# ahcorde/visualSLAM_Android

Measured on AMD Instinct MI355X. Metric: frames/sec (TrackFrame+local BA) on 640×480 synthetic, 1/2/4/8 GPU, higher is better.
Workload: dtype f64

## Files before the change

### include/vslam_c.h

```cpp
#ifndef VSLAM_C_H
#define VSLAM_C_H

#include <stddef.h>
#include <stdint.h>

#ifdef __cplusplus
extern "C" {
#endif

#define VSLAM_LEVELS 4

#define VSLAM_OK 0
#define VSLAM_E_INVALID (-1)
#define VSLAM_E_HIP (-2)
#define VSLAM_E_CAPACITY (-3)
#define VSLAM_E_STATE (-4)

#define VSLAM_Q_CAM_INT_RADIUS 1
#define VSLAM_Q_POSE_INT_RESIDUAL 2
#define VSLAM_Q_NONMAX_RIGHT_NEIGHBOUR 4

typedef struct vslam_system vslam_system;

typedef struct vslam_params {
// ... 32 lines not shown
  int bootstrap;
  int ba_sum_order;
  int relocalise;
  double reloc_blur;
  unsigned pvs_shuffle_seed;
  int overlay;
  int keyframe_retire;
} vslam_params;

const char* vslam_last_error(void);
int vslam_default_params(vslam_params* p, int width, int height, int n_streams);

int vslam_create(const vslam_params* p, vslam_system** out);
int vslam_destroy(vslam_system* sys);
int vslam_synchronize(vslam_system* sys);
int vslam_eval_transcendental(int fn, int n, const double* x, double* y, int on_host);
int vslam_eval_select(int form, int n, const double* v, int k, double* out);
int vslam_eval_pose_tail(const double* sums27, const double* pose12, double* update6, double* pose12_out);


int vslam_make_keyframe_lite(vslam_system* sys, const uint8_t* gray, size_t row_stride,
                             size_t stream_stride, int on_device);

int vslam_fast_nonmax(vslam_system* sys);

int vslam_read_level_image(vslam_system* sys, int stream, int level, uint8_t* dst, size_t dst_stride);
int vslam_read_corners(vslam_system* sys, int stream, int level, uint32_t* corners ,
                       int cap, int* n);
int vslam_read_row_lut(vslam_system* sys, int stream, int level, int* lut );
int vslam_read_max_corners(vslam_system* sys, int stream, int level, uint32_t* corners, int* scores,
                           int cap, int* n);

int vslam_make_keyframe_rest(vslam_system* sys, double min_shi_tomasi_score);
int vslam_thin_candidates(vslam_system* sys, int keyframe);
int vslam_read_candidates(vslam_system* sys, int stream, int level, uint32_t* pos, double* score, int cap, int* n);
int vslam_get_keyframe_corners(vslam_system* sys, int stream, int keyframe, int level, uint32_t* corners, int cap, int* n);
int vslam_read_sbi(vslam_system* sys, int stream, uint8_t* small_img, float* tmpl, double rot8[8]);
int vslam_read_keyframe_sbi(vslam_system* sys, int stream, int keyframe, float* tmpl, float* jacs);
int vslam_get_reloc_info(vslam_system* sys, int stream, int out_i[4], double out_d[24]);
int vslam_read_reloc_attempt(vslam_system* sys, int stream, float* cur_tmpl, double* zmssd, int cap);

int vslam_minipatch_sample(vslam_system* sys, int stream, int n, const int* pos_xy, uint8_t* patches , int* ok);
int vslam_minipatch_find(vslam_system* sys, int stream, int n, const uint8_t* patches, int* pos_xy, int range, int max_ssd,
                         int* found);


// ... 182 lines not shown
```

### visualslam_android_amd/capi.py

```python
import threading
import ctypes as C
import os

import numpy as np

LEVELS = 4
N_STAGES = 14
_HERE = os.path.dirname(os.path.abspath(__file__))
LIB_PATH = os.path.join(_HERE, "libvslam_hip.so")

Q_CAM_INT_RADIUS = 1
Q_POSE_INT_RESIDUAL = 2
Q_NONMAX_RIGHT_NEIGHBOUR = 4

DRAW_POINTS = 1
DRAW_TRAILS = 2
DRAW_FAST = 4
DRAW_IN_PLACE = 8
DRAW_ALPHA0 = 16


class VslamError(RuntimeError):
    pass

# ... 42 lines not shown


class PlaneProbe(C.Structure):
    _fields_ = [("have", C.c_int), ("n", C.c_int), ("best_trial", C.c_int), ("reserved", C.c_int), ("sums", C.c_double * 100),
                ("mean", C.c_double * 3), ("normal", C.c_double * 3), ("R", C.c_double * 9), ("t", C.c_double * 3)]


_lib = None

_ip = C.POINTER(C.c_int)
_sys = C.c_void_p
_vp = C.c_void_p
_i, _d, _sz = C.c_int, C.c_double, C.c_size_t
SYMBOLS = {
    "vslam_last_error": (C.c_char_p, []),
    "vslam_default_params": (_i, [C.POINTER(Params), _i, _i, _i]),
    "vslam_create": (_i, [C.POINTER(Params), C.POINTER(_sys)]),
    "vslam_destroy": (_i, [_sys]),
    "vslam_synchronize": (_i, [_sys]),
    "vslam_eval_transcendental": (_i, [_i, _i, _vp, _vp, _i]),
    "vslam_eval_select": (_i, [_i, _i, _vp, _i, _vp]),
    "vslam_eval_pose_tail": (_i, [_vp, _vp, _vp, _vp]),
    "vslam_make_keyframe_lite": (_i, [_sys, _vp, _sz, _sz, _i]),
    "vslam_fast_nonmax": (_i, [_sys]),
    "vslam_read_level_image": (_i, [_sys, _i, _i, _vp, _sz]),
    "vslam_read_corners": (_i, [_sys, _i, _i, _vp, _i, _ip]),
    "vslam_read_row_lut": (_i, [_sys, _i, _i, _vp]),
    "vslam_read_max_corners": (_i, [_sys, _i, _i, _vp, _vp, _i, _ip]),
    "vslam_get_keyframe_corners": (_i, [_sys, _i, _i, _i, _vp, _i, _ip]),
    "vslam_read_sbi": (_i, [_sys, _i, _vp, _vp, _vp]),
    "vslam_read_keyframe_sbi": (_i, [_sys, _i, _i, _vp, _vp]),
    "vslam_get_reloc_info": (_i, [_sys, _i, _vp, _vp]),
    "vslam_read_reloc_attempt": (_i, [_sys, _i, _vp, _vp, _i]),
    "vslam_attempt_recovery": (_i, [_sys]),
    "vslam_make_keyframe_rest": (_i, [_sys, C.c_double]),
    "vslam_thin_candidates": (_i, [_sys, _i]),
    "vslam_read_candidates": (_i, [_sys, _i, _i, _vp, _vp, _i, _ip]),
    "vslam_minipatch_sample": (_i, [_sys, _i, _i, _vp, _vp, _vp]),
    "vslam_minipatch_find": (_i, [_sys, _i, _i, _vp, _vp, _i, _i, _vp]),
    "vslam_add_keyframe": (_i, [_sys, _i]),
    "vslam_map_add_keyframe": (_i, [_sys, _i, _vp, _i, _vp, _sz, _d, _d]),
    "vslam_map_add_keyframes": (_i, [_sys, _i, _i, _vp, _vp, _vp, _sz, _sz, _vp]),
    "vslam_map_add_point": (_i, [_sys, _i, _vp, _i, _i, _i, _i, _vp, _vp]),
    "vslam_map_add_points": (_i, [_sys, _i, _i, _vp, _vp, _vp, _vp, _vp, _vp]),
    "vslam_map_add_measurement": (_i, [_sys, _i, _i, _i, _i, _vp, _i, _i]),
    "vslam_map_add_measurements": (_i, [_sys, _i, _i, _vp, _vp, _vp, _vp, _vp, _vp]),
# ... 156 lines not shown


def eval_transcendental(name, x, on_host=False):
    x = _f64(x).reshape(-1)
    y = np.zeros_like(x)
    _check(load_library().vslam_eval_transcendental(TRANSCENDENTALS.index(name), len(x), x.ctypes.data, y.ctypes.data, int(on_host)))
    return y


def eval_select(v, k, form=0):
    v = _f64(v).reshape(-1)
    out = np.zeros(1)
    _check(load_library().vslam_eval_select(int(form), len(v), v.ctypes.data, int(k), out.ctypes.data))
    return out[0]


def eval_pose_tail(sums27, pose12):
    s, p = _f64(sums27).reshape(27), _f64(pose12).reshape(12)
    up, out = np.zeros(6), np.zeros(12)
    _check(load_library().vslam_eval_pose_tail(s.ctypes.data, p.ctypes.data, up.ctypes.data, out.ctypes.data))
    return up, out


def pvs_permutation(seed, frame, lst, n, keys=None, on_host=False):
    out = np.zeros(max(n, 0), np.int32)
    k = None if keys is None else np.ascontiguousarray(keys, np.uint32)
    assert k is None or len(k) == n
    _check(load_library().vslam_pvs_permutation(seed, frame, lst, n, None if k is None else k.ctypes.data, out.ctypes.data, int(on_host)))
    return out


def _prims(a, per):
    a = np.ascontiguousarray(np.zeros((0, per)) if a is None else a, np.int32).reshape(-1, per)
    return a, (a.ctypes.data if len(a) else None)


def eval_overlay(gray, marks=None, lines=None, discs=None, flags=0, rgba=None, row_stride=None):
    gray = np.ascontiguousarray(gray, np.uint8)
    h, w = gray.shape
    stride = 4 * w if row_stride is None else int(row_stride)
    nbytes = stride * (h - 1) + 4 * w
    if rgba is None:
        out = np.zeros(nbytes, np.uint8)
    else:
        out = np.ascontiguousarray(rgba, np.uint8).reshape(-1).copy()
        assert out.size >= nbytes, (out.size, nbytes)
# ... 57 lines not shown
        idx, g = self._subset(streams, gray)
        _check(self.lib.vslam_make_keyframe_lite_subset(self.h, idx.ctypes.data if len(idx) else None, len(idx),
                                                        g.ctypes.data if len(idx) else None, g.shape[2], g.shape[1] * g.shape[2], 0))
        self.synchronize()

    def make_keyframe_lite_subset_device(self, streams, dev_ptr, row_stride, stream_stride):
        idx = np.ascontiguousarray(streams, dtype=np.int32).reshape(-1)
        _check(self.lib.vslam_make_keyframe_lite_subset(self.h, idx.ctypes.data if len(idx) else None, len(idx), dev_ptr, row_stride, stream_stride, 1))

    def track_frame_subset(self, streams, gray):
        idx, g = self._subset(streams, gray)
        _check(self.lib.vslam_track_frame_subset(self.h, idx.ctypes.data if len(idx) else None, len(idx),
                                                 g.ctypes.data if len(idx) else None, g.shape[2], g.shape[1] * g.shape[2], 0))
        self.synchronize()

    def track_frame_subset_device(self, streams, dev_ptr, row_stride, stream_stride):
        idx = np.ascontiguousarray(streams, dtype=np.int32).reshape(-1)
        _check(self.lib.vslam_track_frame_subset(self.h, idx.ctypes.data if len(idx) else None, len(idx), dev_ptr, row_stride, stream_stride, 1))

    def step_streams(self):
        out = np.zeros(self.S, dtype=np.uint8)
        _check(self.lib.vslam_get_step_streams(self.h, out.ctypes.data))
        return out

    def fast_nonmax(self):
        _check(self.lib.vslam_fast_nonmax(self.h))

    def read_level_image(self, stream, level):
        h, w = self.level_shape(level)
        out = np.empty((h, w), dtype=np.uint8)
        _check(self.lib.vslam_read_level_image(self.h, stream, level, out.ctypes.data, w))
        return out

    def read_corners(self, stream, level):
        cap = self.params.max_corners[level]
        out = np.empty(cap, dtype=np.uint32)
        n = C.c_int(0)
        _check(self.lib.vslam_read_corners(self.h, stream, level, out.ctypes.data, cap, C.byref(n)))
        return out[:n.value].copy()

    def read_row_lut(self, stream, level):
        h, _ = self.level_shape(level)
        out = np.empty(h, dtype=np.int32)
        _check(self.lib.vslam_read_row_lut(self.h, stream, level, out.ctypes.data))
        return out

# ... 501 lines not shown
```

### visualslam_android_amd/csrc/frontend.hip

```cpp
#include "vslam_internal.h"
#include "fast_reject_dev.h"
#include <stdlib.h>
#include <stdio.h>

#define BAND 16
#define HALO 3
#define FE_THREADS 256

struct FeArgs {
  const uint8_t* in; size_t in_sstride; int in_pitch;
  uint8_t* lvl[NLEV]; size_t lvl_sstride[NLEV]; int lvl_pitch[NLEV];
  int w[NLEV], h[NLEV], nchunk[NLEV], thr[NLEV], cap[NLEV];
  unsigned long long* cmask[NLEV];
  int* rowcnt[NLEV];
  int* rowlut[NLEV];
  uint32_t* corners[NLEV];
  int* ncorners;
  int* overflow;
  int band_first[NLEV];
  const int* list;
};
DEVFN int fe_stream_of(const FeArgs& a, int i) { return a.list ? a.list[i] : i; }

__device__ __forceinline__ bool ring_run10(unsigned m16) {
  unsigned m = m16 | (m16 << 16);
  unsigned r2 = m & (m >> 1);
// ... 162 lines not shown
  if ((int)blockIdx.x >= a.band_first[2]) l = 2;
  if ((int)blockIdx.x >= a.band_first[3]) l = 3;
  const int b = blockIdx.x - a.band_first[l], s = fe_stream_of(a, blockIdx.y);
  const int lp = (a.w[l] + 15) & ~15;
  uint8_t* t = lds;
  unsigned long long* mask_lds = (unsigned long long*)(((uintptr_t)(t + (BAND + 2 * HALO) * lp) + 15) & ~(uintptr_t)15);
  unsigned short* cand = (unsigned short*)(mask_lds + BAND * a.nchunk[l]);
  int* ncand = (int*)(cand + FB_ROWS * lp);
  const int y0 = b * BAND;
  stage_rows(t, lp, a.lvl[l] + (size_t)s * a.lvl_sstride[l], a.lvl_pitch[l], a.w[l], a.h[l], y0 - HALO, BAND + 2 * HALO);
  __syncthreads();
  const int nrows = min(BAND, a.h[l] - y0);
  fast_band(t, lp, y0, nrows, a.w[l], a.h[l], a.thr[l], a.nchunk[l],
            a.cmask[l] + (size_t)s * a.h[l] * a.nchunk[l], a.rowcnt[l] + (size_t)s * a.h[l], mask_lds, cand, ncand);
}

#define SL_RMAX 64
#define SL_THREADS 256
#define SL_CAP 1024
#define SL_RING 8
#define SL_AHEAD (SL_RING - 7)

struct SlArgs {
  int w16[NLEV], nb[NLEV], bpw[NLEV], wg_first[NLEV + 1];
  int R[NLEV];
  int S;
};

DEVFN unsigned sl_half2(unsigned wa, unsigned wb) {
  const unsigned q0 = __builtin_amdgcn_perm(wb, wa, 0x05040100u), q1 = __builtin_amdgcn_perm(wb, wa, 0x07060302u);
  return (__builtin_amdgcn_sad_u8(q0, 0u, 2u) >> 2) | ((__builtin_amdgcn_sad_u8(q1, 0u, 2u) >> 2) << 8);
}
DEVFN unsigned sl_half4(unsigned a0, unsigned a1, unsigned b0, unsigned b1) { return sl_half2(a0, b0) | (sl_half2(a1, b1) << 16); }

struct __attribute__((packed, aligned(4))) SlRow3 { unsigned x, y, z; };
DEVFN bool sl_full_test(const uint8_t* img, int pitch, int w, int x, int y, int thr) {
  const int xb = (x - 3) & ~3, o = (x - 3) & 3;
  const int xl = min(xb, w - 12);
  const bool late = xl != xb;
  unsigned A[7], B[7], v0[7], v1[7], v2[7];
  const uint8_t* r = img + (size_t)(y - 3) * pitch + xl;
#pragma unroll
  for (int k = 0; k < 7; k++) {
    const SlRow3 v = *(const SlRow3*)r;
    v0[k] = v.x; v1[k] = v.y; v2[k] = v.z;
    r += pitch;
  }
  asm volatile("" : "+v"(v0[0]), "+v"(v0[1]), "+v"(v0[2]), "+v"(v0[3]), "+v"(v0[4]), "+v"(v0[5]), "+v"(v0[6]),
                    "+v"(v1[0]), "+v"(v1[1]), "+v"(v1[2]), "+v"(v1[3]), "+v"(v1[4]), "+v"(v1[5]), "+v"(v1[6]));
  asm volatile("" : "+v"(v2[0]), "+v"(v2[1]), "+v"(v2[2]), "+v"(v2[3]), "+v"(v2[4]), "+v"(v2[5]), "+v"(v2[6]));
#pragma unroll
  for (int k = 0; k < 7; k++) {
    const unsigned lo = late ? v1[k] : v0[k], mid = late ? v2[k] : v1[k];
    A[k] = __builtin_amdgcn_alignbyte(mid, lo, o);
    B[k] = __builtin_amdgcn_alignbyte(v2[k], mid, o);
  }
  const int c = (A[3] >> 24) & 255u, cb = c + thr, c_b = c - thr;
  unsigned mb = 0, md = 0;
#define SLPIX(k, dx, dy) { const int v = (int)(((dx) <= 0 ? (A[(dy) + 3] >> (8 * ((dx) + 3))) : (B[(dy) + 3] >> (8 * ((dx) - 1)))) & 255u); mb = __builtin_amdgcn_alignbit(mb, (unsigned)(cb - v), 31); md = __builtin_amdgcn_alignbit(md, (unsigned)(v - c_b), 31); }
  SLPIX(15, -1, 3) SLPIX(14, -2, 2) SLPIX(13, -3, 1) SLPIX(12, -3, 0) SLPIX(11, -3, -1) SLPIX(10, -2, -2)
  SLPIX(9, -1, -3) SLPIX(8, 0, -3) SLPIX(7, 1, -3) SLPIX(6, 2, -2) SLPIX(5, 3, -1) SLPIX(4, 3, 0)
  SLPIX(3, 3, 1) SLPIX(2, 2, 2) SLPIX(1, 1, 3) SLPIX(0, 0, 3)
#undef SLPIX
  return ring_run10(mb) || ring_run10(md);
}

template <bool PYR>
__global__ __launch_bounds__(SL_THREADS) __attribute__((amdgpu_waves_per_eu(4, 4))) void k_fast_slide(FeArgs a, SlArgs q) {
  extern __shared__ __align__(16) uint8_t lds[];
  int l = 0;
  if (!PYR) { l = 1; if ((int)blockIdx.x >= q.wg_first[2]) l = 2; if ((int)blockIdx.x >= q.wg_first[3]) l = 3; }
  const int wg = (int)blockIdx.x - (PYR ? 0 : q.wg_first[l]);
  const int w = a.w[l], h = a.h[l], nchunk = a.nchunk[l], thr = a.thr[l];
  const int W16 = q.w16[l], nb = q.nb[l], bpw = q.bpw[l], SL_R = q.R[l], SL_NSTEP = SL_R + 2 * HALO;
  const uint8_t* img = PYR ? a.in : a.lvl[l];
  const size_t sstride = PYR ? a.in_sstride : a.lvl_sstride[l];
  const int pitch = PYR ? a.in_pitch : a.lvl_pitch[l];
  int4* tb = (int4*)lds;
  unsigned short* lists = (unsigned short*)(tb + SL_THREADS);
  unsigned long long* mask = (unsigned long long*)(lists + (SL_THREADS / 64) * SL_CAP);
  const int tid = threadIdx.x, lane = tid & 63, wave = tid >> 6;
  unsigned short* list = lists + wave * SL_CAP;
  const int bl = tid / W16, cg = tid - bl * W16;
  const long gband = (long)wg * bpw + bl;
  const bool active = bl < bpw && gband < (long)q.S * nb;
  const int ord = active ? (int)(gband / nb) : 0, b = active ? (int)(gband - (long)ord * nb) : 0;
  const int s = active ? fe_stream_of(a, ord) : 0;
  const int yb = b * SL_R, x0 = cg * 16;
  tb[tid] = make_int4(s, yb, x0, active ? bl : -1);
  for (int i = tid; i < bpw * SL_R * nchunk; i += SL_THREADS) mask[i] = 0ull;
  __syncthreads();
  const uint8_t* base = img + (size_t)s * sstride + x0;
  unsigned xvalid = 0;
  for (int j = 0; j < 16; j++) if (x0 + j >= HALO && x0 + j < w - HALO) xvalid |= 1u << j;
  if (!active) xvalid = 0;
// ... 430 lines not shown
}

static void fill_fe_args(vslam_system* sys, FeArgs& a) {
  for (int l = 0; l < NLEV; l++) {
    a.lvl[l] = sys->d_lvl[l];
    a.lvl_sstride[l] = (size_t)sys->geom[l].pitch * sys->geom[l].h;
    a.lvl_pitch[l] = sys->geom[l].pitch;
    a.w[l] = sys->geom[l].w; a.h[l] = sys->geom[l].h; a.nchunk[l] = sys->geom[l].nchunk;
    a.thr[l] = sys->geom[l].thr; a.cap[l] = sys->geom[l].cap;
    a.cmask[l] = sys->fr.cmask[l]; a.rowcnt[l] = sys->fr.rowcnt[l]; a.rowlut[l] = sys->fr.rowlut[l];
    a.corners[l] = sys->fr.corners[l];
  }
  a.ncorners = sys->fr.ncorners;
  a.overflow = sys->fr.overflow;
  a.list = nullptr;
}

static bool fe_slide_ok(const vslam_system* sys, const FeArgs& a) {
  static const bool off = getenv("VSLAM_FE_BANDS") != nullptr;
  if (off) return false;
  for (int l = 0; l < NLEV; l++) if ((a.w[l] & 3) || a.w[l] < 16 || a.w[l] > 4096 || a.h[l] < 7) return false;
  return (((uintptr_t)a.in) & 15) == 0 && (a.in_pitch & 15) == 0 && (a.in_sstride & 15) == 0 && a.in_pitch >= ((a.w[0] + 15) & ~15);
}
static void fe_launch_slide(vslam_system* sys, FeArgs& a, hipStream_t fs, int S) {
  SlArgs q;
  q.S = S;
  int nwg[NLEV];
  size_t lds[NLEV];
  const long slots = 4L * (sys->n_cu > 0 ? sys->n_cu : 256);
  for (int l = 0; l < NLEV; l++) { q.w16[l] = (a.w[l] + 15) >> 4; q.bpw[l] = SL_THREADS / q.w16[l]; }
  auto pick = [&](int l0, int l1) {
    long best = -1; int bestR = 32;
    for (int R = 16; R <= SL_RMAX; R += 8) {
      long wgs = 0;
      bool fits = true;
      for (int l = l0; l <= l1; l++) {
        wgs += ((long)S * ((a.h[l] + R - 1) / R) + q.bpw[l] - 1) / q.bpw[l];
        if ((size_t)SL_THREADS * 16 + (size_t)(SL_THREADS / 64) * SL_CAP * 2 + (size_t)q.bpw[l] * R * a.nchunk[l] * 8 > 60000) fits = false;
      }
      if (!fits && R > 16) continue;
      const long cost = ((wgs + slots - 1) / slots) * (R + 2 * HALO);
      if (best < 0 || cost < best) { best = cost; bestR = R; }
    }
    for (int l = l0; l <= l1; l++) q.R[l] = bestR;
  };
  pick(0, 0);
  pick(1, NLEV - 1);
  for (int l = 0; l < NLEV; l++) {
    q.nb[l] = (a.h[l] + q.R[l] - 1) / q.R[l];
    nwg[l] = (int)(((long)S * q.nb[l] + q.bpw[l] - 1) / q.bpw[l]);
    lds[l] = (size_t)SL_THREADS * 16 + (size_t)(SL_THREADS / 64) * SL_CAP * 2 + (size_t)q.bpw[l] * q.R[l] * a.nchunk[l] * 8;
  }
  static const bool dbg = getenv("VSLAM_FE_DEBUG") != nullptr;
  if (dbg) fprintf(stderr, "fe slide: S %d n_cu %d R %d %d %d %d nb %d %d %d %d wgs %d %d %d %d lds %zu %zu %zu %zu\n", S, sys->n_cu, q.R[0], q.R[1], q.R[2], q.R[3],
                   q.nb[0], q.nb[1], q.nb[2], q.nb[3], nwg[0], nwg[1], nwg[2], nwg[3], lds[0], lds[1], lds[2], lds[3]);
  q.wg_first[0] = 0; q.wg_first[1] = 0;
  for (int l = 1; l < NLEV; l++) q.wg_first[l + 1] = q.wg_first[l] + nwg[l];
  size_t lds123 = lds[1]; if (lds[2] > lds123) lds123 = lds[2]; if (lds[3] > lds123) lds123 = lds[3];
  prof_mark(sys, PROF_PYR_FAST0);
  hipLaunchKernelGGL(k_fast_slide<true>, dim3(nwg[0]), dim3(SL_THREADS), lds[0], fs, a, q);
  prof_mark(sys, PROF_FAST_LVL);
  hipLaunchKernelGGL(k_fast_slide<false>, dim3(q.wg_first[NLEV]), dim3(SL_THREADS), lds123, fs, a, q);
}

#define FE_LDS_MAX (160 * 1024)
static int fe_band_lds(const void* kernel, size_t lds) {
  if (lds > FE_LDS_MAX) { vslam_set_error("front end: a band of %zu B does not fit the %d B of LDS", lds, FE_LDS_MAX); return VSLAM_E_INVALID; }
  if (lds > 48 * 1024) HIPCHK(hipFuncSetAttribute(kernel, hipFuncAttributeMaxDynamicSharedMemorySize, (int)lds));
  return VSLAM_OK;
}
static int fe_launch_bands(vslam_system* sys, FeArgs& a, hipStream_t stream, int S, bool marks) {
  const LevelGeom* g = sys->geom;
  const int lp0 = (g[0].w + 15) & ~15, lp1 = (g[1].w + 15) & ~15, lp2 = (g[2].w + 15) & ~15;
  const size_t lds0 = (size_t)(BAND + 2 * HALO) * lp0 + (BAND / 2) * lp1 + (BAND / 4) * lp2 + 16 + (size_t)BAND * g[0].nchunk * 8 + (size_t)FB_ROWS * lp0 * 2 + 16;
  const size_t lds1 = (size_t)(BAND + 2 * HALO) * lp1 + 16 + (size_t)BAND * g[1].nchunk * 8 + (size_t)FB_ROWS * lp1 * 2 + 16;
  int r = fe_band_lds((const void*)k_pyr_fast0, lds0);
  if (!r) r = fe_band_lds((const void*)k_fast_lvl, lds1);
  if (r) return r;
  if (marks) prof_mark(sys, PROF_PYR_FAST0);
  hipLaunchKernelGGL(k_pyr_fast0, dim3((g[0].h + BAND - 1) / BAND, S), dim3(FE_THREADS), lds0, stream, a, lp0, lp1, lp2);
  int nb = 0;
  a.band_first[0] = 0;
  for (int l = 1; l < NLEV; l++) { a.band_first[l] = nb; nb += (g[l].h + BAND - 1) / BAND; }
  if (marks) prof_mark(sys, PROF_FAST_LVL);
  hipLaunchKernelGGL(k_fast_lvl, dim3(nb, S), dim3(FE_THREADS), lds1, stream, a);
// ... 57 lines not shown
  } else {
    if (sys->step_subset) sys->step_in.assign((size_t)sys->S, 1);
    sys->fe_held = nullptr; sys->map.held = nullptr;
  }
  sys->step_subset = subset;
  if (on_device && !subset) {
    a.in = gray; a.in_sstride = stream_stride; a.in_pitch = (int)row_stride;
  } else {
    for (int i = 0; i < S && !on_device; i++) {
      const int s = subset ? streams[i] : i;
      HIPCHK(hipMemcpy2DAsync(sys->d_lvl[0] + (size_t)s * a.lvl_sstride[0], g[0].pitch, gray + (size_t)i * stream_stride,
                              row_stride, g[0].w, g[0].h, hipMemcpyHostToDevice, fs));
    }
    if (on_device && S > 0)
      hipLaunchKernelGGL(k_gather_level0, dim3((g[0].h + GATHER_ROWS - 1) / GATHER_ROWS, S), dim3(FE_THREADS), 0, fs, gray, stream_stride, (int)row_stride,
                         sys->d_lvl[0], a.lvl_sstride[0], g[0].pitch, g[0].w, g[0].h, (const int*)sys->fr.step_list);
    a.in = sys->d_lvl[0]; a.in_sstride = a.lvl_sstride[0]; a.in_pitch = g[0].pitch;
  }
  sys->fr.img[0] = a.in; sys->fr.img_sstride[0] = a.in_sstride; sys->fr.img_pitch[0] = a.in_pitch;
  for (int l = 1; l < NLEV; l++) { sys->fr.img[l] = a.lvl[l]; sys->fr.img_sstride[l] = a.lvl_sstride[l]; sys->fr.img_pitch[l] = a.lvl_pitch[l]; }
  sys->frbuf[b] = sys->fr;

  if (S > 0) {
    if (fe_slide_ok(sys, a)) fe_launch_slide(sys, a, fs, S);
    else { const int r = fe_launch_bands(sys, a, fs, S, true); if (r) return r; }
  }
  prof_mark(sys, PROF_COMPACT);
  if (S > 0) {
    const CpArgs cp = fe_compact_args(a);
    hipLaunchKernelGGL(k_compact, fe_compact_grid(cp, S), dim3(COMPACT_THREADS), 0, fs, a, cp);
  }
  if (sys->p.use_sbi) {
    const FrameDev& last = sys->have_sbi ? sys->frbuf[b ^ 1] : sys->fr;
    int r = VSLAM_OK;
    if (subset) {
      for (int i = 0; i < n && sys->have_sbi; i++)
        if (!sys->sbi_seen[(size_t)streams[i]]) { HIPCHK(hipMemsetAsync(sys->sbi_restart + streams[i], 1, 1, fs)); sys->sbi_restart_pending = true; }
      for (int i = 0; i < n; i++) sys->sbi_seen[(size_t)streams[i]] = 1;
      if (S > 0) r = fe_sbi(sys, last, a.list, S);
      if (!r && sys->have_sbi && S < sys->S) r = fe_sbi_carry(sys, last);
    } else {
      if (!sys->sbi_all_seen) { sys->sbi_seen.assign((size_t)sys->S, 1); sys->sbi_all_seen = true; }
      r = fe_sbi(sys, last, nullptr, S);
    }
    if (r) return r;
    if (sys->sbi_restart_pending && S > 0) { r = fe_sbi_restart(sys); if (r) return r; if (!subset) sys->sbi_restart_pending = false; }
    if (S > 0) sys->have_sbi = true;
// ... 117 lines not shown
```

### visualslam_android_amd/csrc/system.hip

```cpp
#include "vslam_internal.h"
#include <stdarg.h>
#include <stdio.h>
#include <string.h>

static thread_local char g_err[512] = "";

void vslam_set_error(const char* fmt, ...) {
  va_list ap;
  va_start(ap, fmt);
  vsnprintf(g_err, sizeof(g_err), fmt, ap);
  va_end(ap);
}

extern "C" const char* vslam_last_error(void) { return g_err; }

extern "C" int vslam_default_params(vslam_params* p, int width, int height, int n_streams) {
  if (!p || width < 48 || height < 48 || n_streams < 1) { vslam_set_error("default_params: bad size"); return VSLAM_E_INVALID; }
  memset(p, 0, sizeof(*p));
  p->width = width; p->height = height; p->n_streams = n_streams;
  p->fast_threshold[0] = 10; p->fast_threshold[1] = 15; p->fast_threshold[2] = 15; p->fast_threshold[3] = 10;
  p->nonmax_barrier = 10;
  p->patch_size = 11;
  for (int l = 0; l < NLEV; l++) {
    const int n = ((width >> l) * (height >> l)) / 2;
// ... 33 lines not shown
}

static int sys_acquire(vslam_system* sys) {
  const vslam_params* p = &sys->p;
  DevOwner& own = sys->own;
  VCHK(own.stream(&sys->stream));
  hipStream_t q = sys->stream;
  const int S = sys->S;
  {
    int ncu = 0;
    if (hipDeviceGetAttribute(&ncu, hipDeviceAttributeMultiprocessorCount, p->device) == hipSuccess && ncu > 0) sys->n_cu = ncu;
  }
  VCHK(own.stream(&sys->fe_stream));
  for (int b = 0; b < 2; b++) { VCHK(own.event(&sys->ev_fe_done[b], false)); VCHK(own.event(&sys->ev_track_done[b], false)); }
  for (int k = 0; k < 4; k++) VCHK(own.event(&sys->ev_mm[k], true));
  for (int l = 0; l < NLEV; l++) {
    LevelGeom& g = sys->geom[l];
    g.w = p->width >> l; g.h = p->height >> l;
    g.pitch = (g.w + 63) & ~63;
    g.nchunk = (g.w + 63) >> 6;
    g.cap = p->max_corners[l];
    g.thr = p->fast_threshold[l];
  }
  for (int b = 0; b < 2; b++) {
    FrameDev& fr = sys->frbuf[b];
    for (int l = 0; l < NLEV; l++) {
      const LevelGeom& g = sys->geom[l];
      VCHK(own.alloc(&sys->d_lvl_buf[b][l], (size_t)S * g.pitch * g.h, q));
      VCHK(own.alloc(&fr.cmask[l], (size_t)S * g.h * g.nchunk, q));
      VCHK(own.alloc(&fr.rowcnt[l], (size_t)S * g.h, q));
      VCHK(own.alloc(&fr.rowlut[l], (size_t)S * (g.h + 1), q));
      VCHK(own.alloc(&fr.corners[l], (size_t)S * g.cap, q));
      VCHK(own.alloc(&fr.scores[l], (size_t)S * g.cap, q));
      VCHK(own.alloc(&fr.maxcorners[l], (size_t)S * g.cap, q));
      fr.img[l] = sys->d_lvl_buf[b][l];
      fr.img_sstride[l] = (size_t)g.pitch * g.h;
      fr.img_pitch[l] = g.pitch;
    }
    {
      const size_t ns = (size_t)(sys->geom[3].w / 2) * (sys->geom[3].h / 2);
      VCHK(own.alloc(&fr.sbi_small, (size_t)S * ns, q)); VCHK(own.alloc(&fr.sbi_tmpl, (size_t)S * ns, q));
      VCHK(own.alloc(&fr.sbi_jacs, (size_t)S * ns * 2, q)); VCHK(own.alloc(&fr.sbi_rot, (size_t)S * 8, q));
    }
    VCHK(own.alloc(&fr.ncorners, (size_t)S * NLEV, q));
    VCHK(own.alloc(&fr.nmax, (size_t)S * NLEV, q));
    VCHK(own.alloc(&fr.overflow, 1, q));
// ... 310 lines not shown
```

### visualslam_android_amd/csrc/track.hip

```cpp
#include "vslam_internal.h"
#include "patch_dev.h"
#include "pvs_perm.h"

#define TRK_THREADS 256
#define SORT_CAP 4096
static_assert(SORT_CAP == PVS_SORT_CAP, "a level's list (at most max_points entries) fits the permutation's sort buffer");

template <class T>
DEVFN bool td_project(T& td, int& flags, const double* pos, const Pose& pose, const CamModel& cam, CamProj& pr) {
  flags &= ~TDF_IN_IMAGE;
  double c[3];
  pose_xform(pose, pos, c);
  td.cam[0] = c[0]; td.cam[1] = c[1]; td.cam[2] = c[2];
  if (c[2] < 0.001) return false;
  const double implane[2] = {c[0] / c[2], c[1] / c[2]};
  if (implane[0] * implane[0] + implane[1] * implane[1] > cam.largest_radius * cam.largest_radius) return false;
  pr = cam_project(cam, implane[0], implane[1]);
  td.image[0] = pr.im[0]; td.image[1] = pr.im[1];
  if (pr.invalid) return true;
  if (td.image[0] < 0 || td.image[1] < 0 || td.image[0] > cam.size[0] || td.image[1] > cam.size[1]) return true;
  flags |= TDF_IN_IMAGE;
  return true;
}

// ... 1074 lines not shown
  out[15] = SEARCH_N; out[SEARCH_PROF_SLOTS + 15] = SEARCH_K;
  return VSLAM_OK;
}
extern "C" int vslam_debug_pose_prof(unsigned long long* out16, int reset) {
  HIPCHK(hipDeviceSynchronize());
  HIPCHK(hipMemcpyFromSymbol(out16, HIP_SYMBOL(g_pose_prof), sizeof(unsigned long long) * 16));
  if (reset) { unsigned long long z[16] = {0}; HIPCHK(hipMemcpyToSymbol(HIP_SYMBOL(g_pose_prof), z, sizeof(z))); }
  return VSLAM_OK;
}
#endif

int trk_alloc(vslam_system* sys) {
  const vslam_params& p = sys->p;
  const size_t S = sys->S, P = p.max_points, K = p.max_keyframes;
  if (P > SORT_CAP) { vslam_set_error("max_points %d exceeds %d", (int)P, SORT_CAP); return VSLAM_E_INVALID; }
  MapDev& m = sys->map; DevOwner& own = sys->own; hipStream_t q = sys->stream;
  VCHK(own.alloc(&m.pts, S * P, q)); VCHK(own.alloc(&m.td, S * P, q)); VCHK(own.alloc(&m.tmpl, S * P * TMPL_PITCH, q));
  VCHK(own.alloc(&m.kf_meas, S * K * P, q)); VCHK(own.alloc(&m.cur_meas, S * P, q));
  VCHK(own.alloc(&m.kf_pose, S * K, q)); VCHK(own.alloc(&m.kf_fixed, S * K, q)); VCHK(own.alloc(&m.kf_depth, S * K * 2, q));
  for (int l = 0; l < NLEV; l++) VCHK(own.alloc(&m.kf_img[l], S * K * (size_t)sys->geom[l].pitch * sys->geom[l].h, q));
  VCHK(own.alloc(&m.st, S, q)); VCHK(own.alloc(&m.pvs_list, S * NLEV * P, q)); VCHK(own.alloc(&m.search_list, S * P, q)); VCHK(own.alloc(&m.iter_list, S * P, q)); VCHK(own.alloc(&m.pt_level, S * P, q)); VCHK(own.alloc(&m.pt_flags, S * P, q));
  VCHK(own.alloc(&m.pose_ws, S * POSE_WS_COMPS * P, q)); VCHK(own.alloc(&m.pose_wsi, S * 2 * P, q));
  trk_fill_params(p, sys->tp);
  return VSLAM_OK;
}

void cam_fill(CamModel& c, const double cam5[5], double width, double height, int quirks) {
  c.size[0] = width; c.size[1] = height;
  c.focal[0] = c.size[0] * cam5[0]; c.focal[1] = c.size[1] * cam5[1];
  c.center[0] = c.size[0] * cam5[2] - 0.5; c.center[1] = c.size[1] * cam5[3] - 0.5;
  c.w = cam5[4];
  double one_over_2tan = 0;
  if (c.w != 0.0) { c.two_tan = 2.0 * vlm::vtan(c.w / 2.0); one_over_2tan = 1.0 / c.two_tan; c.winv = 1.0 / c.w; c.distortion_enabled = 1.0; }
  else { c.winv = 0; c.two_tan = 0; c.distortion_enabled = 0; }
  double v2[2];
  if (quirks & VSLAM_Q_CAM_INT_RADIUS) {
    int m1 = (int)cam5[2], m2 = (int)(1.0 - cam5[2]);
    v2[0] = (m1 > m2 ? m1 : m2) / cam5[0];
    m1 = (int)cam5[3]; m2 = (int)(1.0 - cam5[3]);
    v2[1] = (m1 > m2 ? m1 : m2) / cam5[1];
  } else {
    v2[0] = (cam5[2] > 1.0 - cam5[2] ? cam5[2] : 1.0 - cam5[2]) / cam5[0];
    v2[1] = (cam5[3] > 1.0 - cam5[3] ? cam5[3] : 1.0 - cam5[3]) / cam5[1];
  }
  const double rr = sqrt(v2[0] * v2[0] + v2[1] * v2[1]);
  c.largest_radius = c.w == 0.0 ? rr : vlm::vtan(rr * c.w) * one_over_2tan;
// ... 153 lines not shown
```

### visualslam_android_amd/csrc/vslam_internal.h

```cpp
#pragma once
#include <hip/hip_runtime.h>
#include <stdint.h>
#include <string>
#include <vector>
#include "../../include/vslam_c.h"
#include "dev_math.h"

#define NLEV VSLAM_LEVELS

void vslam_set_error(const char* fmt, ...);

#define HIPCHK(expr)                                                                         \
  do {                                                                                       \
    hipError_t _e = (expr);                                                                  \
    if (_e != hipSuccess) {                                                                  \
      vslam_set_error("%s:%d: %s -> %s", __FILE__, __LINE__, #expr, hipGetErrorString(_e)); \
      return VSLAM_E_HIP;                                                                    \
    }                                                                                        \
  } while (0)

#define VCHK(expr) do { int _r = (expr); if (_r) return _r; } while (0)

static inline Pose pose_from12(const double* q) { Pose p; for (int i = 0; i < 9; i++) p.R[i] = q[i]; for (int i = 0; i < 3; i++) p.t[i] = q[9 + i]; return p; }
static inline void pose_to12(const Pose& p, double* q) { for (int i = 0; i < 9; i++) q[i] = p.R[i]; for (int i = 0; i < 3; i++) q[9 + i] = p.t[i]; }
// ... 253 lines not shown
  }
};
template <class T> static inline int host_get(hipStream_t q, T* host, const T* dev, size_t n = 1) { HostCopy c(q); VCHK(c.get(host, dev, n)); return c.wait(); }
template <class T> static inline int host_put(hipStream_t q, T* dev, const T* host, size_t n = 1) { HostCopy c(q); VCHK(c.put(dev, host, n)); return c.wait(); }

struct BaSystemWs;

struct vslam_system {
  vslam_params p;
  int S;
  hipStream_t stream = nullptr;
  LevelGeom geom[NLEV];
  FrameDev fr;
  uint8_t* d_lvl[NLEV];
  FrameDev frbuf[2];
  uint8_t* d_lvl_buf[2][NLEV];
  int fr_idx = 0;
  hipStream_t fe_stream = nullptr;
  hipEvent_t ev_fe_done[2] = {nullptr, nullptr}, ev_track_done[2] = {nullptr, nullptr};
  hipStream_t ba_stream = nullptr;
  std::vector<hipStream_t> ba_streams;
  double* grow_implane = nullptr;
  int n_cu = 0;
  std::vector<hipEvent_t> ev_asm, ev_ba;
  long frame_no = 0;
  long ba_token = 0;
  long ba_batch_id = 0;
  int ba_batch_fill = 0;
  std::vector<long> frame_batch;
  std::vector<int> prof_ba_launched;
  long ba_launch_no = 0;
  hipEvent_t ev_mm[4] = {nullptr, nullptr, nullptr, nullptr};
  int mm_lrec = -1;
  DevOwner own;
  bool have_frame;
  bool frame_open = false;
  bool frame_tracked = false;
  bool have_sbi;
  unsigned char* step_stage[2] = {nullptr, nullptr};
  hipEvent_t ev_step_stage[2] = {nullptr, nullptr};
  bool step_stage_used[2] = {false, false};
  bool step_subset = false;
  std::vector<unsigned char> step_in;
  const unsigned char* fe_held = nullptr;
  std::vector<unsigned char> sbi_seen;
  bool sbi_all_seen = false;
// ... 29 lines not shown
  BaSystemWs* ba_ws = nullptr;
  RelocDev reloc = {nullptr, nullptr, nullptr, nullptr, nullptr};
  std::vector<hipEvent_t> prof_ev;
  int prof_cap = 0, prof_frame = 0;
  bool prof_on = false;
};

enum ProfStage : int {
  PROF_PYR_FAST0, PROF_FAST_LVL, PROF_COMPACT, PROF_PVS, PROF_PLAN_COARSE, PROF_SEARCH_COARSE, PROF_POSE_COARSE, PROF_PLAN_FINE,
  PROF_SEARCH_FINE, PROF_POSE_FINE, PROF_ADD_KEYFRAME, PROF_BA_ASSEMBLE, PROF_BA_COMPUTE, PROF_BA_WRITEBACK, PROF_FRAME_END
};
static_assert(PROF_FRAME_END == VSLAM_N_STAGES, "ProfStage names every stage of include/vslam_c.h");
#define PROF_MARKS (VSLAM_N_STAGES + 3)
#define PROF_FE_END (VSLAM_N_STAGES + 1)
#define PROF_BA_END (VSLAM_N_STAGES + 2)
static inline void prof_mark(vslam_system* sys, int k) {
  if (!(sys->prof_on && sys->prof_frame < sys->prof_cap)) return;
  hipStream_t st = sys->stream;
  if (k <= PROF_COMPACT || k == PROF_FE_END) st = sys->fe_stream;
  else if (sys->tp.ba_delay > 0 && (k == PROF_BA_COMPUTE || k == PROF_BA_END)) st = sys->ba_stream;
  (void)hipEventRecord(sys->prof_ev[(size_t)sys->prof_frame * PROF_MARKS + k], st);
}

int fe_make_keyframe_lite(vslam_system* sys, const uint8_t* gray, size_t row_stride, size_t stream_stride,
                          int on_device, const int* streams = nullptr, int n = -1);
int fe_stream_in_step(vslam_system* sys, int stream, const char* who);
int fe_fast_nonmax(vslam_system* sys);
int fe_keyframe_corners(vslam_system* sys, int s, int kf);
int fe_keyframe_rest_gated(vslam_system* sys);
int fe_thin_new_keyframe(vslam_system* sys, int level);
int grow_alloc(vslam_system* sys);
int grow_on_keyframe(vslam_system* sys);
enum IdleRefind : int { REFIND_NEWLY_MADE = 0, REFIND_FAILURE_QUEUE = 1 };
int grow_idle_refind(vslam_system* sys, int mode);
int mm_idle(vslam_system* sys);
int boot_alloc(vslam_system* sys);
int boot_frame(vslam_system* sys);
int grow_copy_corners(vslam_system* sys);
int grow_levels(vslam_system* sys, const int* order, int n);
int ba_launch_add_keyframe(vslam_system* sys);
enum IdleJob : int { IDLE_BA_RECENT = 0, IDLE_REFIND_NEW = 1, IDLE_BA_ALL = 2, IDLE_REFIND_FAILED = 3, IDLE_N_JOBS };
int mm_idle_job(vslam_system* sys, int job);
int fe_sbi(vslam_system* sys, const FrameDev& last, const int* list, int n);
int fe_sbi_carry(vslam_system* sys, const FrameDev& last);
int fe_sbi_restart(vslam_system* sys);
void cam_fill(CamModel& c, const double cam5[5], double width, double height, int quirks);
// ... 63 lines not shown
```

Measured before the change: 538,100.

## Plan FAST strip heights per level using LDS occupancy and wave scheduling model

Replaces the old per-launch strip-height picker, which used one row count for all coarse levels and a fixed 60 KB LDS cap, with a planner. The planner picks rows per level, sizes LDS against the device's per-CU LDS (checked against the occupancy API), and models workgroup slot scheduling to minimise total row steps. Coarse levels are ordered by strip height in the combined launch so longer workgroups start first. It also adds a public plan query, a strip-row override setter and debug residency prints. In exchange it brings more host-side planning code, a cached plan per stream count, and possibly larger LDS allocations.

```diff
diff --git a/include/vslam_c.h b/include/vslam_c.h
--- a/include/vslam_c.h
+++ b/include/vslam_c.h
@@ -78,6 +78,16 @@
 int vslam_make_keyframe_lite(vslam_system* sys, const uint8_t* gray, size_t row_stride,
                              size_t stream_stride, int on_device);
 
+typedef struct vslam_fe_plan {
+  int rows[4];
+  int workgroups[4];
+  int lds_bytes[2];
+  int workgroups_per_cu[2];
+  double row_steps[2];
+} vslam_fe_plan;
+int vslam_frontend_plan(int width, int height, int streams, int n_cu, int lds_per_cu, vslam_fe_plan* out);
+int vslam_set_frontend_strip_rows(vslam_system* sys, const int rows[4]);
+
 int vslam_fast_nonmax(vslam_system* sys);
 
 int vslam_read_level_image(vslam_system* sys, int stream, int level, uint8_t* dst, size_t dst_stride);
diff --git a/visualslam_android_amd/capi.py b/visualslam_android_amd/capi.py
--- a/visualslam_android_amd/capi.py
+++ b/visualslam_android_amd/capi.py
@@ -88,6 +88,8 @@
     "vslam_eval_select": (_i, [_i, _i, _vp, _i, _vp]),
     "vslam_eval_pose_tail": (_i, [_vp, _vp, _vp, _vp]),
     "vslam_make_keyframe_lite": (_i, [_sys, _vp, _sz, _sz, _i]),
+    "vslam_frontend_plan": (_i, [_i, _i, _i, _i, _i, _vp]),
+    "vslam_set_frontend_strip_rows": (_i, [_sys, _vp]),
     "vslam_fast_nonmax": (_i, [_sys]),
     "vslam_read_level_image": (_i, [_sys, _i, _i, _vp, _sz]),
     "vslam_read_corners": (_i, [_sys, _i, _i, _vp, _i, _ip]),
@@ -290,6 +292,17 @@
     return up, out
 
 
+class FrontendPlan(C.Structure):
+    _fields_ = [("rows", C.c_int * LEVELS), ("workgroups", C.c_int * LEVELS), ("lds_bytes", C.c_int * 2), ("workgroups_per_cu", C.c_int * 2),
+                ("row_steps", C.c_double * 2)]
+
+
+def frontend_plan(width, height, streams, n_cu, lds_per_cu):
+    out = FrontendPlan()
+    _check(load_library().vslam_frontend_plan(width, height, streams, n_cu, lds_per_cu, C.byref(out)))
+    return out
+
+
 def pvs_permutation(seed, frame, lst, n, keys=None, on_host=False):
     out = np.zeros(max(n, 0), np.int32)
     k = None if keys is None else np.ascontiguousarray(keys, np.uint32)
@@ -393,6 +406,10 @@
         out = np.zeros(self.S, dtype=np.uint8)
         _check(self.lib.vslam_get_step_streams(self.h, out.ctypes.data))
         return out
+
+    def set_frontend_strip_rows(self, rows):
+        r = (C.c_int * LEVELS)(*[int(x) for x in rows])
+        _check(self.lib.vslam_set_frontend_strip_rows(self.h, r))
 
     def fast_nonmax(self):
         _check(self.lib.vslam_fast_nonmax(self.h))
diff --git a/visualslam_android_amd/csrc/frontend.hip b/visualslam_android_amd/csrc/frontend.hip
--- a/visualslam_android_amd/csrc/frontend.hip
+++ b/visualslam_android_amd/csrc/frontend.hip
@@ -2,6 +2,8 @@
 #include "fast_reject_dev.h"
 #include <stdlib.h>
 #include <stdio.h>
+#include <utility>
+#include <vector>
 
 #define BAND 16
 #define HALO 3
@@ -210,8 +212,9 @@
 #define SL_AHEAD (SL_RING - 7)
 
 struct SlArgs {
-  int w16[NLEV], nb[NLEV], bpw[NLEV], wg_first[NLEV + 1];
+  int w16[NLEV], nb[NLEV], bpw[NLEV];
   int R[NLEV];
+  int seg_first[NLEV], seg_lev[NLEV - 1];
   int S;
 };
 
@@ -256,9 +259,13 @@
 template <bool PYR>
 __global__ __launch_bounds__(SL_THREADS) __attribute__((amdgpu_waves_per_eu(4, 4))) void k_fast_slide(FeArgs a, SlArgs q) {
   extern __shared__ __align__(16) uint8_t lds[];
-  int l = 0;
-  if (!PYR) { l = 1; if ((int)blockIdx.x >= q.wg_first[2]) l = 2; if ((int)blockIdx.x >= q.wg_first[3]) l = 3; }
-  const int wg = (int)blockIdx.x - (PYR ? 0 : q.wg_first[l]);
+  int l = 0, wg = (int)blockIdx.x;
+  if (!PYR) {
+    int g = 0;
+    if ((int)blockIdx.x >= q.seg_first[1]) g = 1;
+    if ((int)blockIdx.x >= q.seg_first[2]) g = 2;
+    l = q.seg_lev[g]; wg -= q.seg_first[g];
+  }
   const int w = a.w[l], h = a.h[l], nchunk = a.nchunk[l], thr = a.thr[l];
   const int W16 = q.w16[l], nb = q.nb[l], bpw = q.bpw[l], SL_R = q.R[l], SL_NSTEP = SL_R + 2 * HALO;
   const uint8_t* img = PYR ? a.in : a.lvl[l];
@@ -735,45 +742,186 @@
   for (int l = 0; l < NLEV; l++) if ((a.w[l] & 3) || a.w[l] < 16 || a.w[l] > 4096 || a.h[l] < 7) return false;
   return (((uintptr_t)a.in) & 15) == 0 && (a.in_pitch & 15) == 0 && (a.in_sstride & 15) == 0 && a.in_pitch >= ((a.w[0] + 15) & ~15);
 }
-static void fe_launch_slide(vslam_system* sys, FeArgs& a, hipStream_t fs, int S) {
+#define SL_MAX_WG_PER_CU 4
+#define SL_LDS_GRANULE 1280
+static int sl_w16(int w) { return (w + 15) >> 4; }
+static int sl_bpw(int w) { return SL_THREADS / sl_w16(w); }
+static long sl_lds(int w, int R) {
+  return (long)SL_THREADS * 16 + (long)(SL_THREADS / 64) * SL_CAP * 2 + (long)sl_bpw(w) * R * ((w + 63) >> 6) * 8;
+}
+static long sl_nwg(int w, int h, int S, int R) { return ((long)S * ((h + R - 1) / R) + sl_bpw(w) - 1) / sl_bpw(w); }
+static int sl_wg_per_cu(long lds, long lds_per_cu, int max_wg_per_cu) {
+  const long alloc = (lds + SL_LDS_GRANULE - 1) / SL_LDS_GRANULE * SL_LDS_GRANULE;
+  if (lds > lds_per_cu) return 0;
+  const long k = alloc <= lds_per_cu ? lds_per_cu / alloc : 1;
+  return (int)(k < max_wg_per_cu ? k : max_wg_per_cu);
+}
+static double sl_row_steps(long slots, int nseg, const long* n, const int* len) {
+  std::vector<std::pair<long, long>> fr(1, std::make_pair(0L, slots));
+  long end = 0;
+  for (int g = 0; g < nseg; g++) {
+    long left = n[g];
+    while (left > 0) {
+      const long t = fr[0].first, k = fr[0].second < left ? fr[0].second : left;
+      fr[0].second -= k;
+      if (fr[0].second == 0) fr.erase(fr.begin());
+      left -= k;
+      const long t1 = t + len[g];
+      size_t i = 0;
+      while (i < fr.size() && fr[i].first < t1) i++;
+      if (i < fr.size() && fr[i].first == t1) fr[i].second += k; else fr.insert(fr.begin() + i, std::make_pair(t1, k));
+      if (t1 > end) end = t1;
+    }
+  }
+  return (double)end;
+}
+static bool sl_rows_ok(int R) { return R >= 16 && R <= SL_RMAX && (R & 7) == 0; }
+static void sl_order(const int* R, int* ord) {
+  ord[0] = 1; ord[1] = 2; ord[2] = 3;
+  for (int i = 1; i < 3; i++) for (int j = i; j > 0 && R[ord[j]] > R[ord[j - 1]]; j--) { const int t = ord[j]; ord[j] = ord[j - 1]; ord[j - 1] = t; }
+}
+static bool sl_plan(const int* w, const int* h, int S, int n_cu, long lds_per_cu, int max_wg_per_cu, const int* force, vslam_fe_plan* out) {
+  const int l0[2] = {0, 1}, l1[2] = {0, NLEV - 1};
+  for (int launch = 0; launch < 2; launch++) {
+    const int nl = l1[launch] - l0[launch] + 1;
+    double best = -1.0;
+    int R[NLEV], cnt[3] = {0, 0, 0};
+    for (;;) {
+      bool ok = true;
+      long lds = 0;
+      for (int i = 0; i < nl; i++) {
+        const int l = l0[launch] + i;
+        R[l] = 16 + 8 * cnt[i];
+        if (force && force[l] && force[l] != R[l]) ok = false;
+        const long b = sl_lds(w[l], R[l]);
+        if (b > lds) lds = b;
+      }
+      const int wpc = ok ? sl_wg_per_cu(lds, lds_per_cu, max_wg_per_cu) : 0;
+      if (wpc > 0) {
+        int ord[3] = {0, 0, 0};
+        if (launch) sl_order(R, ord);
+        long n[3]; int len[3];
+        for (int i = 0; i < nl; i++) { const int l = ord[i]; n[i] = sl_nwg(w[l], h[l], S, R[l]); len[i] = R[l] + 2 * HALO; }
+        const double cost = sl_row_steps((long)wpc * n_cu, nl, n, len);
+        if (best < 0.0 || cost < best) {
+          best = cost;
+          for (int i = 0; i < nl; i++) { const int l = l0[launch] + i; out->rows[l] = R[l]; out->workgroups[l] = (int)sl_nwg(w[l], h[l], S, R[l]); }
+          out->lds_bytes[launch] = (int)lds; out->workgroups_per_cu[launch] = wpc; out->row_steps[launch] = cost;
+        }
+      }
+      int i = nl - 1;
+      while (i >= 0 && ++cnt[i] > (SL_RMAX - 16) / 8) cnt[i--] = 0;
+      if (i < 0) break;
+    }
+    if (best < 0.0) return false;
+  }
+  return true;
+}
+static bool sl_size_ok(const int* w, const int* h) {
+  for (int l = 0; l < NLEV; l++) if ((w[l] & 3) || w[l] < 16 || w[l] > 4096 || h[l] < 7) return false;
+  return true;
+}
+extern "C" int vslam_frontend_plan(int width, int height, int streams, int n_cu, int lds_per_cu, vslam_fe_plan* out) {
+  if (!out || streams < 1 || n_cu < 1 || lds_per_cu < 1 || width < 1 || height < 1) { vslam_set_error("frontend_plan: bad arguments"); return VSLAM_E_INVALID; }
+  int w[NLEV], h[NLEV];
+  for (int l = 0; l < NLEV; l++) { w[l] = width >> l; h[l] = height >> l; }
+  if (!sl_size_ok(w, h)) { vslam_set_error("frontend_plan: %dx%d is not a size of the strip form", width, height); return VSLAM_E_INVALID; }
+  if (!sl_plan(w, h, streams, n_cu, lds_per_cu, SL_MAX_WG_PER_CU, nullptr, out)) {
+    vslam_set_error("frontend_plan: no strip height fits %d B of LDS", lds_per_cu);
+    return VSLAM_E_INVALID;
+  }
+  return VSLAM_OK;
+}
+
+static int fe_band_lds(const void* kernel, size_t lds);
+static int fe_slide_plan(vslam_system* sys, int S, vslam_fe_plan* out) {
+  for (const auto& e : sys->fe_plans) if (e.first == S) { *out = e.second; return VSLAM_OK; }
+  int w[NLEV], h[NLEV];
+  for (int l = 0; l < NLEV; l++) { w[l] = sys->geom[l].w; h[l] = sys->geom[l].h; }
+  if (!sl_plan(w, h, S, sys->n_cu > 0 ? sys->n_cu : 256, sys->fe_lds_per_cu, SL_MAX_WG_PER_CU, sys->fe_rows, out)) {
+    vslam_set_error("front end: no strip height fits %d B of LDS", sys->fe_lds_per_cu);
+    return VSLAM_E_INVALID;
+  }
+  if (sys->fe_plans.size() >= 64) sys->fe_plans.clear();
+  sys->fe_plans.push_back(std::make_pair(S, *out));
+  return VSLAM_OK;
+}
+int fe_plan_init(vslam_system* sys) {
+  int w[NLEV], h[NLEV];
+  for (int l = 0; l < NLEV; l++) { w[l] = sys->geom[l].w; h[l] = sys->geom[l].h; }
+  if (!sl_size_ok(w, h)) return VSLAM_OK;
+  int lds_cu = 0;
+  if (hipDeviceGetAttribute(&lds_cu, hipDeviceAttributeMaxSharedMemoryPerMultiprocessor, sys->p.device) == hipSuccess && lds_cu > 0) sys->fe_lds_per_cu = lds_cu;
+  static const bool dbg = getenv("VSLAM_FE_DEBUG") != nullptr;
+  for (int it = 0; it < 4; it++) {
+    vslam_fe_plan pl;
+    sys->fe_plans.clear();
+    VCHK(fe_slide_plan(sys, sys->S, &pl));
+    bool same = true;
+    for (int launch = 0; launch < 2; launch++) {
+      const void* k = launch ? (const void*)k_fast_slide<false> : (const void*)k_fast_slide<true>;
+      VCHK(fe_band_lds(k, (size_t)pl.lds_bytes[launch]));
+      int q = 0;
+      if (hipOccupancyMaxActiveBlocksPerMultiprocessor(&q, k, SL_THREADS, (size_t)pl.lds_bytes[launch]) != hipSuccess || q < 1) { (void)hipGetLastError(); continue; }
+      if (q > SL_MAX_WG_PER_CU) q = SL_MAX_WG_PER_CU;
+      if (dbg) fprintf(stderr, "fe plan: launch %d lds %d B, workgroups per CU planned %d, occupancy query %d (LDS per CU %d)\n", launch, pl.lds_bytes[launch],
+                       pl.workgroups_per_cu[launch], q, sys->fe_lds_per_cu);
+      if (q == pl.workgroups_per_cu[launch]) continue;
+      same = false;
+      const long alloc = ((long)pl.lds_bytes[launch] + SL_LDS_GRANULE - 1) / SL_LDS_GRANULE * SL_LDS_GRANULE;
+      sys->fe_lds_per_cu = (int)(q < pl.workgroups_per_cu[launch] ? (long)pl.workgroups_per_cu[launch] * alloc - 1 : (long)q * alloc);
+    }
+    if (same) break;
+  }
+  if (dbg) {
+    int nb = 0;
+    hipFuncAttributes fa;
+    if (hipOccupancyMaxActiveBlocksPerMultiprocessor(&nb, (const void*)k_compact, COMPACT_THREADS, 0) == hipSuccess && hipFuncGetAttributes(&fa, (const void*)k_compact) == hipSuccess)
+      fprintf(stderr, "residency: k_compact threads %d static LDS %zu B registers %d workgroups per CU %d\n", COMPACT_THREADS, fa.sharedSizeBytes, fa.numRegs, nb);
+    else (void)hipGetLastError();
+  }
+  return VSLAM_OK;
+}
+extern "C" int vslam_set_frontend_strip_rows(vslam_system* sys, const int rows[4]) {
+  if (!sys || !rows) { vslam_set_error("set_frontend_strip_rows: null argument"); return VSLAM_E_INVALID; }
+  for (int l = 0; l < NLEV; l++) if (rows[l] != 0 && !sl_rows_ok(rows[l])) {
+    vslam_set_error("set_frontend_strip_rows: level %d: %d rows (0, or a multiple of 8 in 16..%d)", l, rows[l], SL_RMAX);
+    return VSLAM_E_INVALID;
+  }
+  int old[NLEV];
+  for (int l = 0; l < NLEV; l++) { old[l] = sys->fe_rows[l]; sys->fe_rows[l] = rows[l]; }
+  sys->fe_plans.clear();
+  vslam_fe_plan pl;
+  int w[NLEV], h[NLEV];
+  for (int l = 0; l < NLEV; l++) { w[l] = sys->geom[l].w; h[l] = sys->geom[l].h; }
+  const int r = sl_size_ok(w, h) ? fe_slide_plan(sys, sys->S, &pl) : VSLAM_OK;
+  if (r) { for (int l = 0; l < NLEV; l++) sys->fe_rows[l] = old[l]; sys->fe_plans.clear(); }
+  return r;
+}
+
+static int fe_launch_slide(vslam_system* sys, FeArgs& a, hipStream_t fs, int S) {
+  vslam_fe_plan pl;
+  VCHK(fe_slide_plan(sys, S, &pl));
   SlArgs q;
   q.S = S;
-  int nwg[NLEV];
-  size_t lds[NLEV];
-  const long slots = 4L * (sys->n_cu > 0 ? sys->n_cu : 256);
-  for (int l = 0; l < NLEV; l++) { q.w16[l] = (a.w[l] + 15) >> 4; q.bpw[l] = SL_THREADS / q.w16[l]; }
-  auto pick = [&](int l0, int l1) {
-    long best = -1; int bestR = 32;
-    for (int R = 16; R <= SL_RMAX; R += 8) {
-      long wgs = 0;
-      bool fits = true;
-      for (int l = l0; l <= l1; l++) {
-        wgs += ((long)S * ((a.h[l] + R - 1) / R) + q.bpw[l] - 1) / q.bpw[l];
-        if ((size_t)SL_THREADS * 16 + (size_t)(SL_THREADS / 64) * SL_CAP * 2 + (size_t)q.bpw[l] * R * a.nchunk[l] * 8 > 60000) fits = false;
-      }
-      if (!fits && R > 16) continue;
-      const long cost = ((wgs + slots - 1) / slots) * (R + 2 * HALO);
-      if (best < 0 || cost < best) { best = cost; bestR = R; }
-    }
-    for (int l = l0; l <= l1; l++) q.R[l] = bestR;
-  };
-  pick(0, 0);
-  pick(1, NLEV - 1);
   for (int l = 0; l < NLEV; l++) {
+    q.w16[l] = sl_w16(a.w[l]); q.bpw[l] = sl_bpw(a.w[l]); q.R[l] = pl.rows[l];
     q.nb[l] = (a.h[l] + q.R[l] - 1) / q.R[l];
-    nwg[l] = (int)(((long)S * q.nb[l] + q.bpw[l] - 1) / q.bpw[l]);
-    lds[l] = (size_t)SL_THREADS * 16 + (size_t)(SL_THREADS / 64) * SL_CAP * 2 + (size_t)q.bpw[l] * q.R[l] * a.nchunk[l] * 8;
-  }
+  }
+  sl_order(q.R, q.seg_lev);
+  q.seg_first[0] = 0;
+  for (int g = 0; g < NLEV - 1; g++) q.seg_first[g + 1] = q.seg_first[g] + pl.workgroups[q.seg_lev[g]];
   static const bool dbg = getenv("VSLAM_FE_DEBUG") != nullptr;
-  if (dbg) fprintf(stderr, "fe slide: S %d n_cu %d R %d %d %d %d nb %d %d %d %d wgs %d %d %d %d lds %zu %zu %zu %zu\n", S, sys->n_cu, q.R[0], q.R[1], q.R[2], q.R[3],
-                   q.nb[0], q.nb[1], q.nb[2], q.nb[3], nwg[0], nwg[1], nwg[2], nwg[3], lds[0], lds[1], lds[2], lds[3]);
-  q.wg_first[0] = 0; q.wg_first[1] = 0;
-  for (int l = 1; l < NLEV; l++) q.wg_first[l + 1] = q.wg_first[l] + nwg[l];
-  size_t lds123 = lds[1]; if (lds[2] > lds123) lds123 = lds[2]; if (lds[3] > lds123) lds123 = lds[3];
+  if (dbg) fprintf(stderr, "fe slide: S %d n_cu %d R %d %d %d %d nb %d %d %d %d wgs %d %d %d %d lds %d %d per CU %d %d row steps %.1f %.1f\n", S, sys->n_cu, q.R[0], q.R[1], q.R[2], q.R[3],
+                   q.nb[0], q.nb[1], q.nb[2], q.nb[3], pl.workgroups[0], pl.workgroups[1], pl.workgroups[2], pl.workgroups[3], pl.lds_bytes[0], pl.lds_bytes[1],
+                   pl.workgroups_per_cu[0], pl.workgroups_per_cu[1], pl.row_steps[0], pl.row_steps[1]);
+  if (pl.lds_bytes[0] > 48 * 1024) VCHK(fe_band_lds((const void*)k_fast_slide<true>, (size_t)pl.lds_bytes[0]));
+  if (pl.lds_bytes[1] > 48 * 1024) VCHK(fe_band_lds((const void*)k_fast_slide<false>, (size_t)pl.lds_bytes[1]));
   prof_mark(sys, PROF_PYR_FAST0);
-  hipLaunchKernelGGL(k_fast_slide<true>, dim3(nwg[0]), dim3(SL_THREADS), lds[0], fs, a, q);
+  hipLaunchKernelGGL(k_fast_slide<true>, dim3(pl.workgroups[0]), dim3(SL_THREADS), (size_t)pl.lds_bytes[0], fs, a, q);
   prof_mark(sys, PROF_FAST_LVL);
-  hipLaunchKernelGGL(k_fast_slide<false>, dim3(q.wg_first[NLEV]), dim3(SL_THREADS), lds123, fs, a, q);
+  hipLaunchKernelGGL(k_fast_slide<false>, dim3(q.seg_first[NLEV - 1]), dim3(SL_THREADS), (size_t)pl.lds_bytes[1], fs, a, q);
+  return VSLAM_OK;
 }
 
 #define FE_LDS_MAX (160 * 1024)
@@ -877,7 +1025,7 @@
   sys->frbuf[b] = sys->fr;
 
   if (S > 0) {
-    if (fe_slide_ok(sys, a)) fe_launch_slide(sys, a, fs, S);
+    if (fe_slide_ok(sys, a)) { const int r = fe_launch_slide(sys, a, fs, S); if (r) return r; }
     else { const int r = fe_launch_bands(sys, a, fs, S, true); if (r) return r; }
   }
   prof_mark(sys, PROF_COMPACT);
diff --git a/visualslam_android_amd/csrc/system.hip b/visualslam_android_amd/csrc/system.hip
--- a/visualslam_android_amd/csrc/system.hip
+++ b/visualslam_android_amd/csrc/system.hip
@@ -79,6 +79,7 @@
     g.cap = p->max_corners[l];
     g.thr = p->fast_threshold[l];
   }
+  VCHK(fe_plan_init(sys));
   for (int b = 0; b < 2; b++) {
     FrameDev& fr = sys->frbuf[b];
     for (int l = 0; l < NLEV; l++) {
diff --git a/visualslam_android_amd/csrc/track.hip b/visualslam_android_amd/csrc/track.hip
--- a/visualslam_android_amd/csrc/track.hip
+++ b/visualslam_android_amd/csrc/track.hip
@@ -1120,6 +1120,16 @@
   VCHK(own.alloc(&m.st, S, q)); VCHK(own.alloc(&m.pvs_list, S * NLEV * P, q)); VCHK(own.alloc(&m.search_list, S * P, q)); VCHK(own.alloc(&m.iter_list, S * P, q)); VCHK(own.alloc(&m.pt_level, S * P, q)); VCHK(own.alloc(&m.pt_flags, S * P, q));
   VCHK(own.alloc(&m.pose_ws, S * POSE_WS_COMPS * P, q)); VCHK(own.alloc(&m.pose_wsi, S * 2 * P, q));
   trk_fill_params(p, sys->tp);
+  if (getenv("VSLAM_FE_DEBUG")) {
+    const struct { const char* name; const void* k; int threads; } ks[] = {
+      {"k_pvs", (const void*)k_pvs, TRK_THREADS}, {"k_pose", (const void*)k_pose, POSE_THREADS}, {"k_searchN<8,8>", (const void*)k_searchN<8, 8>, 64}};
+    for (const auto& e : ks) {
+      int nb = 0;
+      hipFuncAttributes fa;
+      if (hipOccupancyMaxActiveBlocksPerMultiprocessor(&nb, e.k, e.threads, 0) != hipSuccess || hipFuncGetAttributes(&fa, e.k) != hipSuccess) { (void)hipGetLastError(); continue; }
+      fprintf(stderr, "residency: %s threads %d static LDS %zu B registers %d workgroups per CU %d\n", e.name, e.threads, fa.sharedSizeBytes, fa.numRegs, nb);
+    }
+  }
   return VSLAM_OK;
 }
 
diff --git a/visualslam_android_amd/csrc/vslam_internal.h b/visualslam_android_amd/csrc/vslam_internal.h
--- a/visualslam_android_amd/csrc/vslam_internal.h
+++ b/visualslam_android_amd/csrc/vslam_internal.h
@@ -299,6 +299,9 @@
   std::vector<hipStream_t> ba_streams;
   double* grow_implane = nullptr;
   int n_cu = 0;
+  int fe_lds_per_cu = 160 * 1024;
+  int fe_rows[NLEV] = {0, 0, 0, 0};
+  std::vector<std::pair<int, vslam_fe_plan>> fe_plans;
   std::vector<hipEvent_t> ev_asm, ev_ba;
   long frame_no = 0;
   long ba_token = 0;
@@ -374,6 +377,7 @@
   (void)hipEventRecord(sys->prof_ev[(size_t)sys->prof_frame * PROF_MARKS + k], st);
 }
 
+int fe_plan_init(vslam_system* sys);
 int fe_make_keyframe_lite(vslam_system* sys, const uint8_t* gray, size_t row_stride, size_t stream_stride,
                           int on_device, const int* streams = nullptr, int n = -1);
 int fe_stream_in_step(vslam_system* sys, int stream, const char* who);
```

After: 540,400, median of 6. About the same (+0.4%).
